# Greketrotny/RayZath

Hardware: AMD Instinct MI355X
Metric: Mrays/s (path segments, primary+secondary) at 1920x1080 depth 8 (higher is better)
Workload: dtype f32; 1 GPU; Cornell box 1920x1080 depth 8; max_depth=8, triangles=16, instances=8, traversal=workgroup-binned, integrator=CPU kernel (parity-checked), pipeline=resident (one kernel per step)

## Files before the change

### rayzath_amd/csrc/hiprz_device.hpp

```cpp
#pragma once
#include <hip/hip_runtime.h>
#include <stdint.h>

#include "hiprz.h"
#include "hiprz_end.hpp"
#include "hiprz_lds.hpp"
#include "hiprz_shard.hpp"

#define RZ_DEV __device__ __forceinline__
#include "hiprz_flat_pick.hpp"
#include "hiprz_deal_pick.hpp"
#include "hiprz_pair_pick.hpp"
#include "hiprz_u8_div.hpp"

namespace hiprz {

#ifndef RZ_FUSED_SHARED_RCP
#define RZ_FUSED_SHARED_RCP 0
#endif
#ifndef RZ_TRACE_SHARED_RCP
#define RZ_TRACE_SHARED_RCP 1
#endif
#ifndef RZ_BATCH_SHARED_RCP
#define RZ_BATCH_SHARED_RCP 1
// ... 230 lines not shown
    if (t <= r.near_ || t >= r.far_) return false;
    t_out = t, b1_out = b1, b2_out = b2, det_out = det;
    return true;
}

struct Instance {
    v3 position, scale, xa, ya, za, bb_min, bb_max;
    uint32_t blas_root, material_base, material_count;
};
RZ_DEV void load_instance_box(const DScene& s, uint32_t i, float4& b0, float4& b1) {
    b0 = s.instances[7 * i + 5];
    b1 = s.instances[7 * i + 6];
}
struct InstanceXform {
    v3 position, scale, xa, ya, za;
    uint32_t blas_root;
    bool unit_scale;
};
RZ_DEV InstanceXform load_instance_xform(const DScene& s, uint32_t i) {
    const float4 a = s.instances[7 * i + 0], b = s.instances[7 * i + 1], c = s.instances[7 * i + 2],
                 d = s.instances[7 * i + 3], e = s.instances[7 * i + 4];
    InstanceXform x;
    x.position = xyz(a), x.blas_root = __float_as_uint(a.w);
    x.scale = xyz(b);
    x.unit_scale = __float_as_uint(d.w) != 0u;
    x.xa = xyz(c), x.ya = xyz(d), x.za = xyz(e);
    return x;
}
RZ_DEV v3 transform_forward(v3 xa, v3 ya, v3 za, v3 v) { return xa * v.x + ya * v.y + za * v.z; }
RZ_DEV v3 transform_backward(v3 xa, v3 ya, v3 za, v3 v) {
    return v3{xa.x * v.x + xa.y * v.y + xa.z * v.z, ya.x * v.x + ya.y * v.y + ya.z * v.z,
              za.x * v.x + za.y * v.y + za.z * v.z};
}
RZ_DEV float to_local(const InstanceXform& x, const Ray& g, Ray& l) {
    l.o = g.o - x.position;
    l.o = transform_backward(x.xa, x.ya, x.za, l.o);
    l.o = l.o / x.scale;
    l.d = transform_backward(x.xa, x.ya, x.za, g.d);
    l.d = l.d / x.scale;
    const float len = magnitude(l.d);
    l.near_ = g.near_ * len;
    l.far_ = g.far_ * len;
    l.d = normalized(l.d);
    return len;
}

struct Hit {
    int32_t instance;
    uint32_t triangle;
    float bx, by;
    bool external;
};


typedef float f2 __attribute__((ext_vector_type(2)));
RZ_DEV float refined_rcp(float d) {
    const float r = __builtin_amdgcn_rcpf(d);
    const float e = __builtin_fmaf(-d, r, 1.0f);
    return __builtin_fmaf(e, r, r);
}
RZ_DEV float div_shared(float n, float d, float y) {
    float q = n * y;
    float r = __builtin_fmaf(-d, q, n);
    q = __builtin_fmaf(r, y, q);
    r = __builtin_fmaf(-d, q, n);
    return __builtin_fmaf(r, y, q);
}
RZ_DEV f2 div_shared2(f2 n, float d, float y) {
    const f2 nd = {-d, -d}, yy = {y, y};
    f2 q = n * yy;
    f2 r = __builtin_elementwise_fma(nd, q, n);
    q = __builtin_elementwise_fma(r, yy, q);
    r = __builtin_elementwise_fma(nd, q, n);
    return __builtin_elementwise_fma(r, yy, q);
}
RZ_DEV bool exponent_in(float x, int lo, int hi) {
    const uint32_t e = (__float_as_uint(x) >> 23) & 0xFFu;
    return (e - uint32_t(lo + 127)) < uint32_t(hi - lo);
}
RZ_DEV bool zero_or_exponent_in(float x, int lo, int hi) {
    return (__float_as_uint(x) & 0x7FFFFFFFu) == 0u || exponent_in(x, lo, hi);
}
#ifdef RZ_PHASE_STATS
static __device__ unsigned long long rz_phase[32];
#define RZ_PHASE(k)                                                                                        \
    do {                                                                                                   \
        const unsigned long long rz_a = __ballot(1);                                                       \
        if (int(__builtin_amdgcn_mbcnt_hi(~0u, __builtin_amdgcn_mbcnt_lo(~0u, 0u))) == __ffsll((long long)rz_a) - 1) { \
            atomicAdd(&rz_phase[2 * (k)], 1ull);                                                           \
            atomicAdd(&rz_phase[2 * (k) + 1], (unsigned long long)__popcll(rz_a));                         \
        }                                                                                                  \
    } while (0)
#else
#define RZ_PHASE(k)
#endif
struct WalkRay {
    v3 o, d, y;
    float near_, far_;
    bool fast;
};
template <bool SHARED_RCP>
RZ_DEV void prepare(WalkRay& r, bool scene_fast) {
    if constexpr (!SHARED_RCP) {
        r.fast = false;
        return;
    }
    r.fast = scene_fast && exponent_in(r.d.x, -40, 2) && exponent_in(r.d.y, -40, 2) && exponent_in(r.d.z, -40, 2) &&
             zero_or_exponent_in(r.o.x, -60, 40) && zero_or_exponent_in(r.o.y, -60, 40) && zero_or_exponent_in(r.o.z, -60, 40);
    r.y = v3{refined_rcp(r.d.x), refined_rcp(r.d.y), refined_rcp(r.d.z)};
}
RZ_DEV float vmin(float a, float b) {
    float r;
    asm("v_min_f32 %0, %1, %2" : "=v"(r) : "v"(a), "v"(b));
    return r;
}
RZ_DEV float vmax(float a, float b) {
    float r;
    asm("v_max_f32 %0, %1, %2" : "=v"(r) : "v"(a), "v"(b));
    return r;
}
RZ_DEV float vmin3(float a, float b, float c) {
    float r;
    asm("v_min3_f32 %0, %1, %2, %3" : "=v"(r) : "v"(a), "v"(b), "v"(c));
    return r;
}
RZ_DEV float vmax3(float a, float b, float c) {
    float r;
    asm("v_max3_f32 %0, %1, %2, %3" : "=v"(r) : "v"(a), "v"(b), "v"(c));
    return r;
}
template <bool SHARED_RCP>
RZ_DEV void box_range_unpacked(float4 b0, float4 b1, const WalkRay& r, float& tmin, float& tmax) {
    if (SHARED_RCP && __all(r.fast)) {
        const float t1 = div_shared(b0.x - r.o.x, r.d.x, r.y.x), t2 = div_shared(b0.y - r.o.x, r.d.x, r.y.x);
        const float t3 = div_shared(b0.z - r.o.y, r.d.y, r.y.y), t4 = div_shared(b0.w - r.o.y, r.d.y, r.y.y);
        const float t5 = div_shared(b1.x - r.o.z, r.d.z, r.y.z), t6 = div_shared(b1.y - r.o.z, r.d.z, r.y.z);
        tmin = vmax3(vmin(t1, t2), vmin(t3, t4), vmin(t5, t6));
        tmax = vmin3(vmax(t1, t2), vmax(t3, t4), vmax(t5, t6));
        return;
    }
    const float t1 = (b0.x - r.o.x) / r.d.x;
    const float t2 = (b0.y - r.o.x) / r.d.x;
    const float t3 = (b0.z - r.o.y) / r.d.y;
    const float t4 = (b0.w - r.o.y) / r.d.y;
    const float t5 = (b1.x - r.o.z) / r.d.z;
    const float t6 = (b1.y - r.o.z) / r.d.z;
    tmin = max_gt(max_gt(min_lt(t1, t2), min_lt(t3, t4)), min_lt(t5, t6));
    tmax = min_lt(min_lt(max_gt(t1, t2), max_gt(t3, t4)), max_gt(t5, t6));
}
RZ_DEV void box_range_fast(float4 b0, float4 b1, const WalkRay& r, float& tmin, float& tmax) {
    const float t1 = div_shared(b0.x - r.o.x, r.d.x, r.y.x), t2 = div_shared(b0.y - r.o.x, r.d.x, r.y.x);
    const float t3 = div_shared(b0.z - r.o.y, r.d.y, r.y.y), t4 = div_shared(b0.w - r.o.y, r.d.y, r.y.y);
    const float t5 = div_shared(b1.x - r.o.z, r.d.z, r.y.z), t6 = div_shared(b1.y - r.o.z, r.d.z, r.y.z);
    tmin = vmax3(vmin(t1, t2), vmin(t3, t4), vmin(t5, t6));
    tmax = vmin3(vmax(t1, t2), vmax(t3, t4), vmax(t5, t6));
}
template <bool SHARED_RCP>
RZ_DEV bool box_hit_unpacked(float4 b0, float4 b1, const WalkRay& r) {
    float tmin, tmax;
    box_range_unpacked<SHARED_RCP>(b0, b1, r, tmin, tmax);
    return !(tmax < r.near_ || tmin > tmax || tmin > r.far_);
}
#ifndef RZ_FILTERED_BOX_TEST
#define RZ_FILTERED_BOX_TEST 1
#endif
RZ_DEV void box_filter(float4 b0, float4 b1, const WalkRay& r, bool& missed, bool& hit) {
    const float a1 = (b0.x - r.o.x) * r.y.x, a2 = (b0.y - r.o.x) * r.y.x;
// ... 209 lines not shown
    while (n != RZ_END) {
        RZ_GUARD(guard);
        const float4 n0 = s.nodes[2 * n], n1 = s.nodes[2 * n + 1];
        RZ_COUNT(box_tests);
        RZ_COUNT(shadow_box_tests);
        if (box_hit<false>(n0, n1, g)) {
            const uint32_t begin = __float_as_uint(n1.z), meta = __float_as_uint(n1.w);
            if (!(meta & HIPRZ_NODE_LEAF)) {
                n = w.descend(begin);
                continue;
            }
            const uint32_t end = begin + (meta & HIPRZ_NODE_COUNT_MASK);
            for (uint32_t i = begin; i < end; ++i) {
                const uint32_t inst = s.tlas_order[i];
                float4 ib0, ib1;
                load_instance_box(s, inst, ib0, ib1);
                RZ_COUNT(box_tests);
        RZ_COUNT(shadow_box_tests);
                if (!box_hit<false>(ib0, ib1, g)) continue;
                const InstanceXform x = load_instance_xform(s, inst);
                WalkRay lr;
                to_local<false>(x, g, lr, scene_fast);
                const uint32_t base = w.mark();
                uint32_t m = x.blas_root;
                while (m != RZ_END) {
                    RZ_GUARD(guard);
                    const float4 m0 = s.nodes[2 * m], m1 = s.nodes[2 * m + 1];
                    RZ_COUNT(box_tests);
        RZ_COUNT(shadow_box_tests);
                    if (box_hit<false>(m0, m1, lr)) {
                        const uint32_t mbegin = __float_as_uint(m1.z), mmeta = __float_as_uint(m1.w);
                        if (!(mmeta & HIPRZ_NODE_LEAF)) {
                            m = w.descend(mbegin);
                            continue;
                        }
                        const uint32_t mend = mbegin + (mmeta & HIPRZ_NODE_COUNT_MASK);
                        for (uint32_t j = mbegin; j < mend; ++j) {
                            const float4 a = s.tris[3 * j], b = s.tris[3 * j + 1], c = s.tris[3 * j + 2];
                            float t, b1, b2, det;
                            RZ_COUNT(tri_tests);
                            RZ_COUNT(shadow_tri_tests);
                            if (tri_hit(xyz(a), xyz(b), xyz(c), lr, t, b1, b2, det)) return 0.0f;
                        }
                    }
                    m = w.next(base);
                }
            }
        } else if (n == s.tlas_root) {
            return 1.0f;
        }
        n = w.next(0u);
    }
    return 1.0f;
}


#define RZ_BIN_NONE 0xFFFFFFFFu
#define RZ_BIN_WIDE 0x80000000u
RZ_DEV uint32_t octet_min(uint32_t v);
struct BinnedLds {
    float* ray;
    uint32_t* hit;
    uint32_t* items;
    uint32_t* bins;
    uint32_t* stacks;
    static constexpr uint32_t kFixedBytes = kBinnedFixedBytes;
    static __host__ uint32_t bytes_host(uint32_t world_entries, uint32_t mesh_entries) {
        return kFixedBytes + (world_entries + mesh_entries) * kBinnedEntryBytes;
    }
    __device__ __forceinline__ explicit BinnedLds(unsigned char* base) {
        ray = reinterpret_cast<float*>(base);
        hit = reinterpret_cast<uint32_t*>(base + 8u * 1024u);
        items = reinterpret_cast<uint32_t*>(base + 13u * 1024u);
        bins = reinterpret_cast<uint32_t*>(base + 14u * 1024u);
        stacks = reinterpret_cast<uint32_t*>(base + kFixedBytes);
    }
};

struct FlatWorld {
    float4 root0, root1;
    uint32_t ids;
    uint32_t count;
    uint32_t wide;
};
RZ_DEV uint32_t wave_uniform(uint32_t v) { return uint32_t(__builtin_amdgcn_readfirstlane(int(v))); }
RZ_DEV float wave_uniform(float v) { return __uint_as_float(wave_uniform(__float_as_uint(v))); }
RZ_DEV float4 wave_uniform(float4 v) { return make_float4(wave_uniform(v.x), wave_uniform(v.y), wave_uniform(v.z), wave_uniform(v.w)); }
RZ_DEV FlatWorld make_flat_world(const DScene& s) {
    FlatWorld fw;
    fw.root0 = fw.root1 = make_float4(0.0f, 0.0f, 0.0f, 0.0f);
    fw.ids = fw.count = fw.wide = 0u;
    if (s.n_instances == 0) return fw;
    fw.root0 = wave_uniform(s.nodes[2 * s.tlas_root]), fw.root1 = wave_uniform(s.nodes[2 * s.tlas_root + 1]);
    const uint32_t begin = __float_as_uint(fw.root1.z);
    fw.count = __float_as_uint(fw.root1.w) & HIPRZ_NODE_COUNT_MASK;
    if (fw.count > 8u) fw.count = 8u;
#pragma unroll
    for (uint32_t k = 0; k < 8u; ++k)
        if (k < fw.count) fw.ids = flat_pack_id(fw.ids, k, wave_uniform(s.tlas_order[begin + k]));
    const uint32_t i = threadIdx.x & 63u;
    bool wide = false;
    if (i < s.n_instances && i < 8u) {
        const uint32_t root = __float_as_uint(s.instances[7 * i].w);
        const uint32_t meta = __float_as_uint(s.nodes[2 * root + 1].w);
        wide = (meta & HIPRZ_NODE_LEAF) != 0u && (meta & HIPRZ_NODE_COUNT_MASK) > 4u;
    }
    fw.wide = uint32_t(__ballot(wide)) & 0xFFu;
    return fw;
}

template <bool COUNT, bool RCP>
RZ_DEV uint32_t pretest_leaf_instances(const DScene& s, const FlatWorld& fw, const WalkRay& g, float (&tm)[8], bool counting, Counters& cnt) {
    uint32_t mask = 0u;
    if (fw.count == 8u && RCP && __all(g.fast)) {
#pragma unroll
        for (uint32_t k = 0; k < 8u; ++k) {
            float4 ib0, ib1;
            load_instance_box(s, flat_id(fw.ids, k), ib0, ib1);
            float tmin, tmax;
            box_range_fast(ib0, ib1, g, tmin, tmax);
            if (counting) { RZ_PHASE(1); RZ_COUNT(box_tests); }
            mask |= uint32_t(!(tmax < g.near_ || tmin > tmax)) << k;
            tm[k] = tmin;
        }
        return mask;
    }
#pragma unroll
    for (uint32_t k = 0; k < 8u; ++k) {
        tm[k] = 0.0f;
        if (k < fw.count) {
            float4 ib0, ib1;
            load_instance_box(s, flat_id(fw.ids, k), ib0, ib1);
            float tmin, tmax;
            box_range_unpacked<RCP>(ib0, ib1, g, tmin, tmax);
            if (counting) { RZ_PHASE(1); RZ_COUNT(box_tests); }
            mask |= uint32_t(!(tmax < g.near_ || tmin > tmax)) << k;
            tm[k] = tmin;
        }
    }
    return mask;
}

RZ_DEV uint32_t lane_pull(uint32_t from_lane, uint32_t v) { return uint32_t(__builtin_amdgcn_ds_bpermute(int(from_lane << 2), int(v))); }
RZ_DEV float lane_pull(uint32_t from_lane, float v) { return __uint_as_float(lane_pull(from_lane, __float_as_uint(v))); }
template <int N>
RZ_DEV uint32_t row_below(uint32_t v) {
    return uint32_t(__builtin_amdgcn_update_dpp(0, int(v), 0x110 + N, 0xF, 0xF, true));
}
RZ_DEV uint32_t wave_inclusive_sum(uint32_t v, uint32_t lane) {
    v += row_below<1>(v), v += row_below<2>(v), v += row_below<4>(v), v += row_below<8>(v);
    const uint32_t r0 = uint32_t(__builtin_amdgcn_readlane(int(v), 15)), r1 = uint32_t(__builtin_amdgcn_readlane(int(v), 31));
    const uint32_t r2 = uint32_t(__builtin_amdgcn_readlane(int(v), 47));
    return v + (lane >= 16u ? r0 : 0u) + (lane >= 32u ? r1 : 0u) + (lane >= 48u ? r2 : 0u);
}
RZ_DEV void dealt_hit(const BinnedLds& lds, uint32_t item, float near_, float len, const LeafBest& best) {
    const uint32_t inst = item >> 8, src = item & 255u;
    lds.ray[6 * 256 + src] = near_ / len;
    lds.ray[7 * 256 + src] = best.far_ / len;
    lds.hit[0 * 256 + src] = best.triangle;
    lds.hit[1 * 256 + src] = best.external ? 1u : 0u;
    lds.hit[2 * 256 + src] = __float_as_uint(best.b1);
    lds.hit[3 * 256 + src] = __float_as_uint(best.b2);
    lds.hit[4 * 256 + src] = inst;
}
template <bool COUNT, bool RCP>
RZ_DEV bool dealt_visit(const DScene& s, const BinnedLds& lds, bool scene_fast, uint32_t slot, bool has_item, Counters& cnt) {
    const uint32_t lane = threadIdx.x & 63u;
    const unsigned char* section = pair_section(s);
    uint32_t item = 0u, rec_off = 0u, begin = 0u, count = 0u, n_pairs = 0u, p = 0u;
    WalkRay lr;
    lr.o = lr.d = lr.y = V3(0.0f, 0.0f, 0.0f), lr.near_ = lr.far_ = 0.0f, lr.fast = false;
    float len = 1.0f;
    bool inner = false;
    if (has_item) {
        item = lds.items[slot];
        const uint32_t inst = item >> 8, src = item & 255u;
        WalkRay w;
        w.o = V3(lds.ray[0 * 256 + src], lds.ray[1 * 256 + src], lds.ray[2 * 256 + src]);
        w.d = V3(lds.ray[3 * 256 + src], lds.ray[4 * 256 + src], lds.ray[5 * 256 + src]);
        w.near_ = lds.ray[6 * 256 + src], w.far_ = lds.ray[7 * 256 + src];
        const InstanceXform x = load_instance_xform(s, inst);
        const float4 n0 = s.nodes[2 * x.blas_root], n1 = s.nodes[2 * x.blas_root + 1];
        inner = (__float_as_uint(n1.w) & HIPRZ_NODE_LEAF) == 0u;
        if (!inner) {
            RZ_PHASE(2);
            len = to_local<RCP>(x, w, lr, scene_fast);
            RZ_PHASE(3);
            RZ_COUNT(box_tests);
            if (box_hit_unpacked<RCP>(n0, n1, lr)) {
                begin = __float_as_uint(n1.z), count = __float_as_uint(n1.w) & HIPRZ_NODE_COUNT_MASK, n_pairs = (count + 1u) >> 1;
// ... 72 lines not shown
        best.far_ = __uint_as_float(nearest);
        best.triangle = won ? won_triangle & ~kDealExternal : 0xFFFFFFFFu;
        best.external = (won_triangle & kDealExternal) != 0u;
        best.b1 = won_b1, best.b2 = won_b2;
        lr.near_ = own_near;
    }
    if (best.triangle != 0xFFFFFFFFu) dealt_hit(lds, item, lr.near_, len, best);
    return inner;
}
template <bool COUNT, bool RCP>
RZ_DEV void binned_visit(const DScene& s, const BinnedLds& lds, uint32_t* mesh_column, bool scene_fast, uint32_t slot, Counters& cnt) {
    RZ_PHASE(2);
    const uint32_t item = lds.items[slot], inst = (item & 0x7FFFFFFFu) >> 8, src = item & 255u;
    WalkRay w;
    w.o = V3(lds.ray[0 * 256 + src], lds.ray[1 * 256 + src], lds.ray[2 * 256 + src]);
    w.d = V3(lds.ray[3 * 256 + src], lds.ray[4 * 256 + src], lds.ray[5 * 256 + src]);
    w.near_ = lds.ray[6 * 256 + src], w.far_ = lds.ray[7 * 256 + src];
    const InstanceXform x = load_instance_xform(s, inst);
    WalkRay lr;
    const float len = to_local<RCP>(x, w, lr, scene_fast);
    const float4 n0 = s.nodes[2 * x.blas_root], n1 = s.nodes[2 * x.blas_root + 1];
    const bool wide = (item & RZ_BIN_WIDE) != 0u;
    if (wide || (__float_as_uint(n1.w) & HIPRZ_NODE_LEAF) != 0u) {
        const uint32_t j = wide ? slot & 7u : 0u;
        RZ_PHASE(3);
        if (j == 0u) { RZ_COUNT(box_tests); }
        LeafBest best;
        best.far_ = lr.far_, best.triangle = 0xFFFFFFFFu, best.b1 = best.b2 = 0.0f, best.external = false;
        if (box_hit_unpacked<RCP>(n0, n1, lr)) {
            const uint32_t begin = __float_as_uint(n1.z), end = begin + (__float_as_uint(n1.w) & HIPRZ_NODE_COUNT_MASK);
            const uint32_t count = end - begin, n_pairs = (count + 1u) >> 1;
            const unsigned char* section = pair_section(s);
            const float2* rec = reinterpret_cast<const float2*>(section + 8u * reinterpret_cast<const uint16_t*>(section)[inst]);
            for (uint32_t p = j; p < n_pairs; p += wide ? 8u : 1u) {
                const float2* q = rec + p * (RZ_PAIR_RECORD_BYTES / 8u);
                const float2 v1x = q[0], v1y = q[1], v1z = q[2], e1x = q[3], e1y = q[4], e1z = q[5], e2x = q[6], e2y = q[7], e2z = q[8];
                const bool has_b = 2u * p + 1u < count;
                const uint32_t i = begin + 2u * p;
                RZ_PHASE(4);
#ifdef RZ_PHASE_STATS
                if (!wide && p >= 1u) { RZ_PHASE(9); }
                if (!wide && p == 1u) {
                    const uint32_t k = uint32_t(__popcll(__ballot(1)));
                    RZ_PHASE(10);
                    if (k <= 12u) { RZ_PHASE(11); } else if (k <= 25u) { RZ_PHASE(12); } else { RZ_PHASE(13); }
                }
#endif
                if constexpr (COUNT) cnt.tri_tests += has_b ? 2u : 1u;
                tri_pair_step(v3p{f2{v1x.x, v1x.y}, f2{v1y.x, v1y.y}, f2{v1z.x, v1z.y}}, v3p{f2{e1x.x, e1x.y}, f2{e1y.x, e1y.y}, f2{e1z.x, e1z.y}},
                              v3p{f2{e2x.x, e2x.y}, f2{e2y.x, e2y.y}, f2{e2z.x, e2z.y}}, i, has_b, lr, best);
            }
        }
        bool mine = best.triangle != 0xFFFFFFFFu;
        if (wide) {
            const uint32_t wide_t = mine ? __float_as_uint(best.far_) : 0xFFFFFFFFu;
            const uint32_t t_min = octet_min(wide_t);
            const bool nearest = wide_t != 0xFFFFFFFFu && wide_t == t_min;
            const uint32_t first = octet_min(nearest ? best.triangle : 0xFFFFFFFFu);
            mine = nearest && best.triangle == first;
        }
        if (mine) {
            lds.ray[6 * 256 + src] = lr.near_ / len;
            lds.ray[7 * 256 + src] = best.far_ / len;
            lds.hit[0 * 256 + src] = best.triangle;
            lds.hit[1 * 256 + src] = best.external ? 1u : 0u;
            lds.hit[2 * 256 + src] = __float_as_uint(best.b1);
            lds.hit[3 * 256 + src] = __float_as_uint(best.b2);
            lds.hit[4 * 256 + src] = inst;
        }
        return;
    }
    LdsStack mesh(mesh_column);
    Hit h;
    if (closest_in_mesh_stack<COUNT, RCP, false>(s, mesh, x.blas_root, lr, h, cnt)) {
        lds.ray[6 * 256 + src] = lr.near_ / len;
        lds.ray[7 * 256 + src] = lr.far_ / len;
        lds.hit[0 * 256 + src] = h.triangle;
        lds.hit[1 * 256 + src] = h.external ? 1u : 0u;
        lds.hit[2 * 256 + src] = __float_as_uint(h.bx);
        lds.hit[3 * 256 + src] = __float_as_uint(h.by);
        lds.hit[4 * 256 + src] = inst;
    }
}

template <bool COUNT, bool RCP>
__device__ __forceinline__ int closest_hit_binned(const DScene& s, unsigned char* workspace, bool active, Ray& ray, Hit& hit,
                                                  Counters& cnt) {
    const uint32_t tid = threadIdx.x;
    BinnedLds lds(workspace);
    hit.instance = -1, hit.triangle = 0, hit.bx = hit.by = 0.0f, hit.external = true;
    if (s.n_instances == 0) return 0;

    lds.ray[0 * 256 + tid] = ray.o.x, lds.ray[1 * 256 + tid] = ray.o.y, lds.ray[2 * 256 + tid] = ray.o.z;
    lds.ray[3 * 256 + tid] = ray.d.x, lds.ray[4 * 256 + tid] = ray.d.y, lds.ray[5 * 256 + tid] = ray.d.z;
    lds.ray[6 * 256 + tid] = ray.near_, lds.ray[7 * 256 + tid] = ray.far_;
    lds.hit[4 * 256 + tid] = 0xFFFFFFFFu;

    LdsStack world(lds.stacks + tid);
    uint32_t* mesh_column = lds.stacks + s.world_stack_entries * 256u + tid;
    const bool sorted = s.n_instances <= 64u;
    WalkRay g;
    g.o = ray.o, g.d = ray.d, g.near_ = ray.near_, g.far_ = ray.far_;
    const bool scene_fast = s.fast_div != 0u;
    prepare<RCP>(g, scene_fast);
    uint32_t n = active ? s.tlas_root : RZ_END;
    uint32_t leaf_i = 0, leaf_end = 0;
    bool root_missed = false;
    uint32_t round = 0u;
    if (tid < 128u) lds.bins[tid] = 0u;
    unsigned long long wide_mask = 0ull;
    if (sorted) {
        const uint32_t k = tid & 63u;
        bool wide = false;
        if (k < s.n_instances) {
            const uint32_t root = __float_as_uint(s.instances[7 * k].w);
            const uint32_t meta = __float_as_uint(s.nodes[2 * root + 1].w);
            wide = (meta & HIPRZ_NODE_LEAF) != 0u && (meta & HIPRZ_NODE_COUNT_MASK) > 4u;
        }
        wide_mask = __ballot(wide);
    }
    __syncthreads();

    uint32_t guard = 0u;
    while (round < (1u << 20)) {
        RZ_PHASE(5);
        uint32_t cand = RZ_BIN_NONE;
        while (true) {
            RZ_GUARD(guard);
            if (leaf_i < leaf_end) {
                const uint32_t inst = s.tlas_order[leaf_i++];
                float4 ib0, ib1;
                load_instance_box(s, inst, ib0, ib1);
                RZ_PHASE(1);
                RZ_COUNT(box_tests);
                if (box_hit_unpacked<RCP>(ib0, ib1, g)) {
                    cand = inst;
                    break;
                }
                continue;
            }
            if (n == RZ_END) break;
            const float4 n0 = s.nodes[2 * n], n1 = s.nodes[2 * n + 1];
            RZ_PHASE(0);
            RZ_COUNT(box_tests);
            if (box_hit_unpacked<RCP>(n0, n1, g)) {
                const uint32_t begin = __float_as_uint(n1.z), meta = __float_as_uint(n1.w);
                if (!(meta & HIPRZ_NODE_LEAF)) {
                    n = world.descend(begin);
                    continue;
                }
                leaf_i = begin, leaf_end = begin + (meta & HIPRZ_NODE_COUNT_MASK);
            } else if (n == s.tlas_root) {
                root_missed = true;
            }
            n = world.next(0u);
        }

        uint32_t* bins = lds.bins + (round & 1u) * 64u;
        uint32_t rank = 0u;
        const uint32_t bin = sorted ? cand : 0u;
        const bool wide_item = cand != RZ_BIN_NONE && cand < 64u && ((wide_mask >> cand) & 1ull) != 0ull;
        if (cand != RZ_BIN_NONE) rank = atomicAdd(&bins[bin], wide_item ? 8u : 1u);
        __syncthreads();
        const uint32_t lane = tid & 63u;
        const uint32_t c = bins[lane];
        const bool wide_bin = ((wide_mask >> lane) & 1ull) != 0ull;
// ... 63 lines not shown
                const uint32_t first = octet_min(nearest ? wide_tri : 0xFFFFFFFFu);
                if (nearest && wide_tri == first) {
                    lds.ray[6 * 256 + src] = visit_near / len;
                    lds.ray[7 * 256 + src] = __uint_as_float(wide_t) / len;
                    lds.hit[0 * 256 + src] = wide_tri;
                    lds.hit[1 * 256 + src] = wide_external ? 1u : 0u;
                    lds.hit[2 * 256 + src] = __float_as_uint(wide_b1);
                    lds.hit[3 * 256 + src] = __float_as_uint(wide_b2);
                    lds.hit[4 * 256 + src] = inst;
                }
            } else {
                LdsStack mesh(mesh_column);
                Hit h;
                if (closest_in_mesh_stack<COUNT, RCP, false>(s, mesh, x.blas_root, lr, h, cnt)) {
                    lds.ray[6 * 256 + src] = lr.near_ / len;
                    lds.ray[7 * 256 + src] = lr.far_ / len;
                    lds.hit[0 * 256 + src] = h.triangle;
                    lds.hit[1 * 256 + src] = h.external ? 1u : 0u;
                    lds.hit[2 * 256 + src] = __float_as_uint(h.bx);
                    lds.hit[3 * 256 + src] = __float_as_uint(h.by);
                    lds.hit[4 * 256 + src] = inst;
                }
            }
        }
        __syncthreads();
        round += 1u;
        g.near_ = lds.ray[6 * 256 + tid];
        g.far_ = lds.ray[7 * 256 + tid];
    }
    ray.o = V3(lds.ray[0 * 256 + tid], lds.ray[1 * 256 + tid], lds.ray[2 * 256 + tid]);
    ray.d = V3(lds.ray[3 * 256 + tid], lds.ray[4 * 256 + tid], lds.ray[5 * 256 + tid]);
    ray.near_ = g.near_, ray.far_ = g.far_;
    const uint32_t inst = lds.hit[4 * 256 + tid];
    if (inst != 0xFFFFFFFFu) {
        hit.instance = int32_t(inst);
        hit.triangle = lds.hit[0 * 256 + tid];
        hit.external = lds.hit[1 * 256 + tid] != 0u;
        hit.bx = __uint_as_float(lds.hit[2 * 256 + tid]);
        hit.by = __uint_as_float(lds.hit[3 * 256 + tid]);
    }
    if (root_missed) return 0;
    return hit.instance >= 0 ? 2 : 1;
}


struct DppShr {
    template <int N>
    __device__ __forceinline__ uint32_t operator()(uint32_t v, FlatShift<N>) const {
        return uint32_t(__builtin_amdgcn_update_dpp(0, int(v), 0x110 + N, 0xF, 0xF, true));
    }
};
template <bool COUNT, bool RCP>
__device__ __forceinline__ int closest_hit_flat(const DScene& s, const FlatWorld& fw, unsigned char* workspace, bool active, Ray& ray, Hit& hit,
                                                Counters& cnt) {
    const uint32_t tid = threadIdx.x;
    BinnedLds lds(workspace);
    hit.instance = -1, hit.triangle = 0, hit.bx = hit.by = 0.0f, hit.external = true;
    if (s.n_instances == 0) return 0;

    lds.ray[0 * 256 + tid] = ray.o.x, lds.ray[1 * 256 + tid] = ray.o.y, lds.ray[2 * 256 + tid] = ray.o.z;
    lds.ray[3 * 256 + tid] = ray.d.x, lds.ray[4 * 256 + tid] = ray.d.y, lds.ray[5 * 256 + tid] = ray.d.z;
    lds.ray[6 * 256 + tid] = ray.near_, lds.ray[7 * 256 + tid] = ray.far_;
    lds.hit[4 * 256 + tid] = 0xFFFFFFFFu;

    uint32_t* mesh_column = lds.stacks + s.world_stack_entries * 256u + tid;
    WalkRay g;
    g.o = ray.o, g.d = ray.d, g.near_ = ray.near_, g.far_ = ray.far_;
    const bool scene_fast = s.fast_div != 0u;
    prepare<RCP>(g, scene_fast);
    bool root_missed = false;
    uint32_t round = 0u;
    float tm[8] = {0.0f, 0.0f, 0.0f, 0.0f, 0.0f, 0.0f, 0.0f, 0.0f};
    uint32_t flat_mask = 0u, flat_next = 0u;
    float flat_near = g.near_;
    if (active) {
        RZ_PHASE(0);
        RZ_COUNT(box_tests);
        if (box_hit_unpacked<RCP>(fw.root0, fw.root1, g)) flat_mask = pretest_leaf_instances<COUNT, RCP>(s, fw, g, tm, true, cnt);
        else root_missed = true;
    }
    if (tid < 128u) lds.bins[tid] = 0u;
    __syncthreads();

    const uint32_t lane = tid & 63u;
    const bool wide_bin = ((fw.wide >> (lane & 7u)) & 1u) != 0u;
    while (round < (1u << 20)) {
        RZ_PHASE(5);
        if (__any(flat_mask != 0u && __float_as_uint(g.near_) != __float_as_uint(flat_near))) {
            if (flat_mask != 0u && __float_as_uint(g.near_) != __float_as_uint(flat_near)) {
                WalkRay t;
                t.o = V3(lds.ray[0 * 256 + tid], lds.ray[1 * 256 + tid], lds.ray[2 * 256 + tid]);
                t.d = V3(lds.ray[3 * 256 + tid], lds.ray[4 * 256 + tid], lds.ray[5 * 256 + tid]);
                t.near_ = g.near_, t.far_ = g.far_;
                prepare<RCP>(t, scene_fast);
                flat_mask = pretest_leaf_instances<COUNT, RCP>(s, fw, t, tm, false, cnt) & flat_from(flat_next);
                flat_near = g.near_;
            }
        }
        const uint32_t cand = flat_pick(fw.ids, tm, g.far_, flat_mask, flat_next);

        uint32_t* bins = lds.bins + (round & 1u) * 64u;
        uint32_t rank = 0u;
        const bool wide_item = cand != kFlatNone && ((fw.wide >> cand) & 1u) != 0u;
        if (cand != kFlatNone) rank = atomicAdd(&bins[cand], wide_item ? 8u : 1u);
        __syncthreads();
        const uint32_t c = bins[lane];
        if (!__any(c != 0u)) break;
        const uint32_t own = flat_pack_bin(c, wide_bin);
        const uint32_t incl = flat_prefix8(own, DppShr{});
        const FlatRound r = flat_round(uint32_t(__builtin_amdgcn_readlane(int(incl), 7)));
#ifdef RZ_PHASE_STATS
        if (!r.split) { RZ_PHASE(6); }
#endif
        const uint32_t before = __shfl(incl - own, int(cand & 7u));
        if (cand != kFlatNone) {
            const uint32_t at = flat_item_slot(r, before, rank, wide_item);
            if (r.split && wide_item) {
#pragma unroll
                for (uint32_t j = 0; j < 8u; ++j) lds.items[at + j] = RZ_BIN_WIDE | (cand << 8) | tid;
            } else {
                lds.items[at] = (cand << 8) | tid;
            }
        }
        if (tid < 64u) lds.bins[((round + 1u) & 1u) * 64u + tid] = 0u;
        __syncthreads();

        const uint32_t slot = (tid - ((blockIdx.x + round) & 3u) * 64u) & 255u;
        const bool has_item = slot < r.n_items;
        bool deal_wave = false;
        if (!r.split && wave_uniform(slot & ~63u) < r.n_items) {
            const bool long_leaf = has_item && ((fw.wide >> (lds.items[has_item ? slot : 0u] >> 8)) & 1u) != 0u;
            const uint32_t owners = uint32_t(__popcll(__ballot(long_leaf)));
            deal_wave = owners != 0u && owners <= kDealMaxOwners;
        }
        bool todo = has_item;
        if (deal_wave) todo = dealt_visit<COUNT, RCP>(s, lds, scene_fast, slot, has_item, cnt);
        if (todo) {
            binned_visit<COUNT, RCP>(s, lds, mesh_column, scene_fast, slot, cnt);
        }
        __syncthreads();
        round += 1u;
        g.near_ = lds.ray[6 * 256 + tid];
        g.far_ = lds.ray[7 * 256 + tid];
    }
    ray.o = V3(lds.ray[0 * 256 + tid], lds.ray[1 * 256 + tid], lds.ray[2 * 256 + tid]);
    ray.d = V3(lds.ray[3 * 256 + tid], lds.ray[4 * 256 + tid], lds.ray[5 * 256 + tid]);
    ray.near_ = g.near_, ray.far_ = g.far_;
    const uint32_t inst = lds.hit[4 * 256 + tid];
    if (inst != 0xFFFFFFFFu) {
        hit.instance = int32_t(inst);
        hit.triangle = lds.hit[0 * 256 + tid];
        hit.external = lds.hit[1 * 256 + tid] != 0u;
        hit.bx = __uint_as_float(lds.hit[2 * 256 + tid]);
        hit.by = __uint_as_float(lds.hit[3 * 256 + tid]);
    }
    if (root_missed) return 0;
    return hit.instance >= 0 ? 2 : 1;
}


struct TopCache {
    const float4* nodes;
    const uint32_t* skip;
    uint32_t count;
    static __host__ uint32_t bytes_host(uint32_t top_count) { return top_count * kTopNodeBytes; }
};
RZ_DEV uint32_t octant_of(v3 d) { return uint32_t(d.z < 0.0f) | (uint32_t(d.y < 0.0f) << 1) | (uint32_t(d.x < 0.0f) << 2); }
RZ_DEV void fetch_node_ordered(const DScene& s, uint32_t n, uint32_t oct, float4& n0, float4& n1, uint32_t& link) {
    const float4* rec = s.nodes64 + 4 * size_t(n);
    n0 = rec[0], n1 = rec[1];
    link = reinterpret_cast<const uint32_t*>(rec + 2)[oct];
}
RZ_DEV bool tri_hit_ordered(v3 v1, v3 edge1, v3 edge2, const WalkRay& r, bool tie_ok, float& t_out, float& b1_out, float& b2_out, float& det_out) {
    const v3 pvec = cross(r.d, edge2);
    float det = dot(edge1, pvec);
    det += float(uint32_t(det > -1.0e-7f) & uint32_t(det < 1.0e-7f)) * 1.0e-7f;
    const float inv_det = 1.0f / det;
    const v3 tvec = r.o - v1;
    const float b1 = dot(tvec, pvec) * inv_det;
    if (b1 < 0.0f || b1 > 1.0f) return false;
    const v3 qvec = cross(tvec, edge1);
    const float b2 = dot(r.d, qvec) * inv_det;
    if (b2 < 0.0f || b1 + b2 > 1.0f) return false;
    const float t = dot(edge2, qvec) * inv_det;
    if (t <= r.near_ || t > r.far_ || (t == r.far_ && !tie_ok)) return false;
    t_out = t, b1_out = b1, b2_out = b2, det_out = det;
    return true;
}
RZ_DEV void fetch_node(const DScene& s, const TopCache& top, uint32_t n, float4& n0, float4& n1, uint32_t& link) {
    if (n < top.count) {
        n0 = top.nodes[2 * n], n1 = top.nodes[2 * n + 1], link = top.skip[n];
    } else {
        n0 = s.nodes[2 * n], n1 = s.nodes[2 * n + 1], link = s.node_skip[n];
    }
}
// ... 1318 lines not shown
```

### rayzath_amd/csrc/hiprz_flat_pick.hpp

```cpp
#pragma once
#include <stdint.h>

#ifndef RZ_DEV
#define RZ_DEV inline
#endif

namespace hiprz {

constexpr uint32_t kFlatNone = 0xFFFFFFFFu;

RZ_DEV uint32_t flat_ctz(uint32_t v) { return uint32_t(__builtin_ctz(v)); }
RZ_DEV uint32_t flat_top_bit(uint32_t v) { return 31u - uint32_t(__builtin_clz(v)); }

RZ_DEV uint32_t flat_pack_id(uint32_t packed, uint32_t k, uint32_t id) { return packed | ((id & 15u) << (4u * k)); }
RZ_DEV uint32_t flat_id(uint32_t packed, uint32_t k) { return (packed >> (4u * k)) & 15u; }
RZ_DEV uint32_t flat_slots(uint32_t count) { return (1u << count) - 1u; }
RZ_DEV uint32_t flat_from(uint32_t next) { return ~((1u << next) - 1u); }

RZ_DEV uint32_t flat_le_mask(const float (&tm)[8], float far_) {
    uint32_t m = 0u;
#pragma unroll
    for (uint32_t k = 0; k < 8u; ++k) m |= uint32_t(!(tm[k] > far_)) << k;
    return m;
}

RZ_DEV uint32_t flat_pick(uint32_t ids, const float (&tm)[8], float far_, uint32_t& mask, uint32_t& next) {
    const uint32_t rest = mask & flat_from(next);
    const uint32_t alive = rest & flat_le_mask(tm, far_);
    if (alive != 0u) {
        const uint32_t k = flat_ctz(alive);
        next = k + 1u;
        return flat_id(ids, k);
    }
    if (rest != 0u) next = flat_top_bit(rest) + 1u;
    mask = 0u;
    return kFlatNone;
}

RZ_DEV uint32_t flat_pack_bin(uint32_t c, bool wide) { return wide ? (c | ((c >> 3) << 21)) : ((c << 12) | (c << 21)); }

template <int N>
struct FlatShift {};
template <class V, class Shr>
RZ_DEV V flat_prefix8(V incl, const Shr& shr) {
    incl += shr(incl, FlatShift<1>{});
    incl += shr(incl, FlatShift<2>{});
    incl += shr(incl, FlatShift<4>{});
    return incl;
}

struct FlatRound {
    uint32_t n_visits, wide_lanes, narrow_lanes, n_items;
    bool split;
};
RZ_DEV FlatRound flat_round(uint32_t totals) {
    FlatRound r;
    r.n_visits = totals >> 21;
    r.wide_lanes = totals & 0xFFFu, r.narrow_lanes = (totals >> 12) & 0x1FFu;
    r.split = r.wide_lanes != 0u && r.wide_lanes + r.narrow_lanes <= 256u;
    r.n_items = r.split ? r.wide_lanes + r.narrow_lanes : r.n_visits;
    return r;
}
RZ_DEV uint32_t flat_item_slot(const FlatRound& r, uint32_t before, uint32_t rank, bool wide_item) {
    if (r.split && wide_item) return (before & 0xFFFu) + rank;
    if (r.split) return r.wide_lanes + ((before >> 12) & 0x1FFu) + rank;
    return (before >> 21) + (wide_item ? rank >> 3 : rank);
}

}
```

### rayzath_amd/csrc/hiprz_launch_shade.hip

```cpp
#include "hiprz_ctx.hpp"
#include "hiprz_kernels.hpp"

#ifndef RZ_PACKET_MINW
#define RZ_PACKET_MINW 4
#endif

namespace hiprz {
namespace {

void sort_after_shading(hiprz_ctx* c, const DFrame& f) {
    launch_sort(c, f.shadow_key != nullptr);
    if (f.shadow_key) launch_shadow_sort(c);
}

template <bool FIRST, bool COUNT>
void launch_shade_t(hiprz_ctx* c, const DFrame& f) {
    const ShadeVariant& v = c->plan.shade;
    const DConfig cfg = make_config(c);
    const dim3 grid(v.grid), block(v.block);
#define RZ_SHADE(L, S) RZ_LAUNCH((rz_shade_kernel<FIRST, COUNT, L, S>), grid, block, v.lds, c->stream, c->dscene, c->dcamera, cfg, f, v.top_n)
    switch (v.shadow) {
        case RZ_SHADOW_COMPAT_DEFER: RZ_SHADE(false, RZ_SHADOW_COMPAT_DEFER); break;
        case RZ_SHADOW_COMPAT: RZ_SHADE(false, RZ_SHADOW_COMPAT); break;
        case RZ_SHADOW_PLAIN:
            if (v.lds_scene) RZ_SHADE(true, RZ_SHADOW_PLAIN);
            else RZ_SHADE(false, RZ_SHADOW_PLAIN);
            break;
        case RZ_SHADOW_NONE:
            if (v.lds_scene) RZ_SHADE(true, RZ_SHADOW_NONE);
            else RZ_SHADE(false, RZ_SHADOW_NONE);
            break;
        case RZ_SHADOW_DEFER: RZ_SHADE(false, RZ_SHADOW_DEFER); break;
        case 1: RZ_SHADE(true, 1); break;
        default: RZ_SHADE(false, 3); break;
    }
#undef RZ_SHADE
    if (v.follow == SHADOWS_NONE) return;
    sort_after_shading(c, f);
    const dim3 sgrid(v.follow_grid), sblock(v.follow_block);
    switch (v.follow) {
        case SHADOWS_PACKET: RZ_LAUNCH((rz_shadow_packet_kernel<FIRST, COUNT, RZ_PACKET_MINW>), sgrid, sblock, v.follow_lds, c->stream, c->dscene, c->dcamera, cfg, f); break;
        case SHADOWS_PACKET_COLOUR: RZ_LAUNCH((rz_shadow_packet_kernel<FIRST, COUNT, RZ_PACKET_MINW, true>), sgrid, sblock, v.follow_lds, c->stream, c->dscene, c->dcamera, cfg, f); break;
        case SHADOWS_COOP3_COLOUR: RZ_LAUNCH((rz_shadow_coop_kernel<FIRST, COUNT, 3, true>), sgrid, sblock, v.follow_lds, c->stream, c->dscene, c->dcamera, cfg, f); break;
        case SHADOWS_COOP4: RZ_LAUNCH((rz_shadow_coop_kernel<FIRST, COUNT, 4>), sgrid, sblock, v.follow_lds, c->stream, c->dscene, c->dcamera, cfg, f); break;
        case SHADOWS_SKIP6: RZ_LAUNCH((rz_shadow_kernel<FIRST, COUNT, 6>), sgrid, sblock, v.follow_lds, c->stream, c->dscene, c->dcamera, cfg, f, v.follow_top_n); break;
        default: RZ_LAUNCH((rz_shadow_kernel<FIRST, COUNT, 4>), sgrid, sblock, v.follow_lds, c->stream, c->dscene, c->dcamera, cfg, f, v.follow_top_n); break;
    }
    join_sort(c);
}

}

void launch_shade(hiprz_ctx* c, const DFrame& f, bool first, bool counted) {
    if (first) counted ? launch_shade_t<true, true>(c, f) : launch_shade_t<true, false>(c, f);
    else counted ? launch_shade_t<false, true>(c, f) : launch_shade_t<false, false>(c, f);
}

}

#ifdef RZ_PHASE_STATS
extern "C" int hiprz_read_shadow_phase_stats(unsigned long long out[32]) {
    (void)hipMemcpyFromSymbol(out, HIP_SYMBOL(hiprz::rz_phase), 256);
    unsigned long long zero[32] = {0};
    (void)hipMemcpyToSymbol(HIP_SYMBOL(hiprz::rz_phase), zero, 256);
    return 0;
}
#endif
```

### rayzath_amd/csrc/hiprz_launch_trace.hip

```cpp
#include "hiprz_ctx.hpp"
#include "hiprz_kernels.hpp"

namespace hiprz {
namespace {

template <bool FIRST, bool COUNT>
void launch_trace_t(hiprz_ctx* c, const DFrame& f) {
    const TraceVariant& t = c->plan.trace;
    const dim3 grid(t.grid), block(t.block);
    if (t.family == TRACE_COMPAT) {
        RZ_LAUNCH((rz_trace_coop_compat_kernel<FIRST, COUNT>), grid, block, t.lds, c->stream, c->dscene, c->dcamera, make_config(c), f);
    } else if (t.family == TRACE_COOP) {
        if (t.waves == 5u && t.one_leaf) RZ_LAUNCH((rz_trace_coop_kernel<FIRST, COUNT, 5, true>), grid, block, t.lds, c->stream, c->dscene, c->dcamera, f);
        else if (t.waves == 5u) RZ_LAUNCH((rz_trace_coop_kernel<FIRST, COUNT, 5>), grid, block, t.lds, c->stream, c->dscene, c->dcamera, f);
        else if (t.waves == 6u) RZ_LAUNCH((rz_trace_coop_kernel<FIRST, COUNT, 6>), grid, block, t.lds, c->stream, c->dscene, c->dcamera, f);
        else if (t.one_leaf) RZ_LAUNCH((rz_trace_coop_kernel<FIRST, COUNT, 4, true>), grid, block, t.lds, c->stream, c->dscene, c->dcamera, f);
        else RZ_LAUNCH((rz_trace_coop_kernel<FIRST, COUNT, 4>), grid, block, t.lds, c->stream, c->dscene, c->dcamera, f);
    } else if (t.family == TRACE_SKIP) {
        if (t.waves == 6u) RZ_LAUNCH((rz_trace_skip_kernel<FIRST, COUNT, 6>), grid, block, t.lds, c->stream, c->dscene, c->dcamera, f, t.top_n);
        else RZ_LAUNCH((rz_trace_skip_kernel<FIRST, COUNT, 4>), grid, block, t.lds, c->stream, c->dscene, c->dcamera, f, t.top_n);
    } else if (t.mode == 4u) {
        RZ_LAUNCH((rz_trace_kernel<FIRST, COUNT, 4, true>), grid, block, t.lds, c->stream, c->dscene, c->dcamera, f);
    } else if (t.mode == 2u) {
        if (t.lds_scene) RZ_LAUNCH((rz_trace_kernel<FIRST, COUNT, 2, true>), grid, block, t.lds, c->stream, c->dscene, c->dcamera, f);
        else RZ_LAUNCH((rz_trace_kernel<FIRST, COUNT, 2, false>), grid, block, t.lds, c->stream, c->dscene, c->dcamera, f);
    } else {
        if (t.lds_scene) RZ_LAUNCH((rz_trace_kernel<FIRST, COUNT, 1, true>), grid, block, t.lds, c->stream, c->dscene, c->dcamera, f);
        else RZ_LAUNCH((rz_trace_kernel<FIRST, COUNT, 1, false>), grid, block, t.lds, c->stream, c->dscene, c->dcamera, f);
    }
}

}

void launch_trace(hiprz_ctx* c, const DFrame& f, bool first, bool counted) {
    if (first) counted ? launch_trace_t<true, true>(c, f) : launch_trace_t<true, false>(c, f);
    else counted ? launch_trace_t<false, true>(c, f) : launch_trace_t<false, false>(c, f);
}

}

#ifdef RZ_PHASE_STATS
extern "C" int hiprz_read_phase_stats(unsigned long long out[32]) {
    (void)hipMemcpyFromSymbol(out, HIP_SYMBOL(hiprz::rz_phase), 256);
    unsigned long long zero[32] = {0};
    (void)hipMemcpyToSymbol(HIP_SYMBOL(hiprz::rz_phase), zero, 256);
    return 0;
}
#endif
```

Measured before the change: 13770 Mrays/s.

## Visit nearest small-leaf instance per-thread before binned traversal

```diff
diff --git a/rayzath_amd/csrc/hiprz_device.hpp b/rayzath_amd/csrc/hiprz_device.hpp
--- a/rayzath_amd/csrc/hiprz_device.hpp
+++ b/rayzath_amd/csrc/hiprz_device.hpp
@@ -336,7 +336,7 @@
     return (__float_as_uint(x) & 0x7FFFFFFFu) == 0u || exponent_in(x, lo, hi);
 }
 #ifdef RZ_PHASE_STATS
-static __device__ unsigned long long rz_phase[32];
+static __device__ unsigned long long rz_phase[40];
 #define RZ_PHASE(k)                                                                                        \
     do {                                                                                                   \
         const unsigned long long rz_a = __ballot(1);                                                       \
@@ -712,6 +712,7 @@
     uint32_t ids;
     uint32_t count;
     uint32_t wide;
+    uint32_t small;
 };
 RZ_DEV uint32_t wave_uniform(uint32_t v) { return uint32_t(__builtin_amdgcn_readfirstlane(int(v))); }
 RZ_DEV float wave_uniform(float v) { return __uint_as_float(wave_uniform(__float_as_uint(v))); }
@@ -719,7 +720,7 @@
 RZ_DEV FlatWorld make_flat_world(const DScene& s) {
     FlatWorld fw;
     fw.root0 = fw.root1 = make_float4(0.0f, 0.0f, 0.0f, 0.0f);
-    fw.ids = fw.count = fw.wide = 0u;
+    fw.ids = fw.count = fw.wide = fw.small = 0u;
     if (s.n_instances == 0) return fw;
     fw.root0 = wave_uniform(s.nodes[2 * s.tlas_root]), fw.root1 = wave_uniform(s.nodes[2 * s.tlas_root + 1]);
     const uint32_t begin = __float_as_uint(fw.root1.z);
@@ -729,13 +730,15 @@
     for (uint32_t k = 0; k < 8u; ++k)
         if (k < fw.count) fw.ids = flat_pack_id(fw.ids, k, wave_uniform(s.tlas_order[begin + k]));
     const uint32_t i = threadIdx.x & 63u;
-    bool wide = false;
+    bool wide = false, small = false;
     if (i < s.n_instances && i < 8u) {
         const uint32_t root = __float_as_uint(s.instances[7 * i].w);
         const uint32_t meta = __float_as_uint(s.nodes[2 * root + 1].w);
         wide = (meta & HIPRZ_NODE_LEAF) != 0u && (meta & HIPRZ_NODE_COUNT_MASK) > 4u;
+        small = (meta & HIPRZ_NODE_LEAF) != 0u && (meta & HIPRZ_NODE_COUNT_MASK) <= 4u;
     }
     fw.wide = uint32_t(__ballot(wide)) & 0xFFu;
+    fw.small = uint32_t(__ballot(small)) & 0xFFu;
     return fw;
 }
 
@@ -974,6 +977,52 @@
         lds.hit[4 * 256 + src] = inst;
     }
 }
+template <bool COUNT, bool RCP>
+RZ_DEV void first_visit(const DScene& s, const BinnedLds& lds, bool scene_fast, uint32_t inst, WalkRay& g, Counters& cnt) {
+    RZ_PHASE(2);
+    const uint32_t src = threadIdx.x;
+    const InstanceXform x = load_instance_xform(s, inst);
+    WalkRay lr;
+    const float len = to_local<RCP>(x, g, lr, scene_fast);
+    const float4 n0 = s.nodes[2 * x.blas_root], n1 = s.nodes[2 * x.blas_root + 1];
+    RZ_PHASE(3);
+    RZ_COUNT(box_tests);
+    LeafBest best;
+    best.far_ = lr.far_, best.triangle = 0xFFFFFFFFu, best.b1 = best.b2 = 0.0f, best.external = false;
+    if (box_hit_unpacked<RCP>(n0, n1, lr)) {
+        const uint32_t begin = __float_as_uint(n1.z), count = __float_as_uint(n1.w) & HIPRZ_NODE_COUNT_MASK, n_pairs = (count + 1u) >> 1;
+        const unsigned char* section = pair_section(s);
+        const float2* rec = reinterpret_cast<const float2*>(section + 8u * reinterpret_cast<const uint16_t*>(section)[inst]);
+        for (uint32_t p = 0u; p < n_pairs; ++p) {
+            const float2* q = rec + p * (RZ_PAIR_RECORD_BYTES / 8u);
+            const float2 v1x = q[0], v1y = q[1], v1z = q[2], e1x = q[3], e1y = q[4], e1z = q[5], e2x = q[6], e2y = q[7], e2z = q[8];
+            const bool has_b = 2u * p + 1u < count;
+            const uint32_t i = begin + 2u * p;
+            RZ_PHASE(4);
+#ifdef RZ_PHASE_STATS
+            if (p >= 1u) {
+                const uint32_t k = uint32_t(__popcll(__ballot(1)));
+                RZ_PHASE(9);
+                RZ_PHASE(10);
+                if (k <= 12u) { RZ_PHASE(11); } else if (k <= 25u) { RZ_PHASE(12); } else { RZ_PHASE(13); }
+            }
+#endif
+            if constexpr (COUNT) cnt.tri_tests += has_b ? 2u : 1u;
+            tri_pair_step(v3p{f2{v1x.x, v1x.y}, f2{v1y.x, v1y.y}, f2{v1z.x, v1z.y}}, v3p{f2{e1x.x, e1x.y}, f2{e1y.x, e1y.y}, f2{e1z.x, e1z.y}},
+                          v3p{f2{e2x.x, e2x.y}, f2{e2y.x, e2y.y}, f2{e2z.x, e2z.y}}, i, has_b, lr, best);
+        }
+    }
+    if (best.triangle != 0xFFFFFFFFu) {
+        g.near_ = lr.near_ / len, g.far_ = best.far_ / len;
+        lds.ray[6 * 256 + src] = g.near_;
+        lds.ray[7 * 256 + src] = g.far_;
+        lds.hit[0 * 256 + src] = best.triangle;
+        lds.hit[1 * 256 + src] = best.external ? 1u : 0u;
+        lds.hit[2 * 256 + src] = __float_as_uint(best.b1);
+        lds.hit[3 * 256 + src] = __float_as_uint(best.b2);
+        lds.hit[4 * 256 + src] = inst;
+    }
+}
 
 template <bool COUNT, bool RCP>
 __device__ __forceinline__ int closest_hit_binned(const DScene& s, unsigned char* workspace, bool active, Ray& ray, Hit& hit,
@@ -1203,6 +1252,21 @@
     if (tid < 128u) lds.bins[tid] = 0u;
     __syncthreads();
 
+#ifdef RZ_PHASE_STATS
+    {
+        uint32_t peek_mask = flat_mask, peek_next = flat_next;
+        const uint32_t peek = flat_pick(fw.ids, tm, g.far_, peek_mask, peek_next);
+        if (peek != kFlatNone) {
+            if (((fw.small >> peek) & 1u) != 0u) { RZ_PHASE(15); } else { RZ_PHASE(16); }
+        }
+    }
+#endif
+    {
+        const uint32_t first = flat_pick_first(fw.ids, tm, g.far_, flat_mask, flat_next, fw.small);
+        if (__any(first != kFlatNone)) {
+            if (first != kFlatNone) first_visit<COUNT, RCP>(s, lds, scene_fast, first, g, cnt);
+        }
+    }
     const uint32_t lane = tid & 63u;
     const bool wide_bin = ((fw.wide >> (lane & 7u)) & 1u) != 0u;
     while (round < (1u << 20)) {
@@ -1232,6 +1296,10 @@
         const FlatRound r = flat_round(uint32_t(__builtin_amdgcn_readlane(int(incl), 7)));
 #ifdef RZ_PHASE_STATS
         if (!r.split) { RZ_PHASE(6); }
+        if (round == 0u) {
+            RZ_PHASE(17);
+            if (!r.split) { RZ_PHASE(18); }
+        }
 #endif
         const uint32_t before = __shfl(incl - own, int(cand & 7u));
         if (cand != kFlatNone) {
diff --git a/rayzath_amd/csrc/hiprz_flat_pick.hpp b/rayzath_amd/csrc/hiprz_flat_pick.hpp
--- a/rayzath_amd/csrc/hiprz_flat_pick.hpp
+++ b/rayzath_amd/csrc/hiprz_flat_pick.hpp
@@ -37,6 +37,20 @@
     return kFlatNone;
 }
 
+RZ_DEV uint32_t flat_pick_first(uint32_t ids, const float (&tm)[8], float far_, uint32_t& mask, uint32_t& next, uint32_t small) {
+    const uint32_t rest = mask & flat_from(next);
+    const uint32_t alive = rest & flat_le_mask(tm, far_);
+    if (alive != 0u) {
+        const uint32_t k = flat_ctz(alive), id = flat_id(ids, k);
+        if (((small >> id) & 1u) == 0u) return kFlatNone;
+        next = k + 1u;
+        return id;
+    }
+    if (rest != 0u) next = flat_top_bit(rest) + 1u;
+    mask = 0u;
+    return kFlatNone;
+}
+
 RZ_DEV uint32_t flat_pack_bin(uint32_t c, bool wide) { return wide ? (c | ((c >> 3) << 21)) : ((c << 12) | (c << 21)); }
 
 template <int N>
diff --git a/rayzath_amd/csrc/hiprz_launch_shade.hip b/rayzath_amd/csrc/hiprz_launch_shade.hip
--- a/rayzath_amd/csrc/hiprz_launch_shade.hip
+++ b/rayzath_amd/csrc/hiprz_launch_shade.hip
@@ -59,10 +59,10 @@
 }
 
 #ifdef RZ_PHASE_STATS
-extern "C" int hiprz_read_shadow_phase_stats(unsigned long long out[32]) {
-    (void)hipMemcpyFromSymbol(out, HIP_SYMBOL(hiprz::rz_phase), 256);
-    unsigned long long zero[32] = {0};
-    (void)hipMemcpyToSymbol(HIP_SYMBOL(hiprz::rz_phase), zero, 256);
+extern "C" int hiprz_read_shadow_phase_stats(unsigned long long out[40]) {
+    (void)hipMemcpyFromSymbol(out, HIP_SYMBOL(hiprz::rz_phase), sizeof(hiprz::rz_phase));
+    unsigned long long zero[40] = {0};
+    (void)hipMemcpyToSymbol(HIP_SYMBOL(hiprz::rz_phase), zero, sizeof(hiprz::rz_phase));
     return 0;
 }
 #endif
diff --git a/rayzath_amd/csrc/hiprz_launch_trace.hip b/rayzath_amd/csrc/hiprz_launch_trace.hip
--- a/rayzath_amd/csrc/hiprz_launch_trace.hip
+++ b/rayzath_amd/csrc/hiprz_launch_trace.hip
@@ -40,10 +40,10 @@
 }
 
 #ifdef RZ_PHASE_STATS
-extern "C" int hiprz_read_phase_stats(unsigned long long out[32]) {
-    (void)hipMemcpyFromSymbol(out, HIP_SYMBOL(hiprz::rz_phase), 256);
-    unsigned long long zero[32] = {0};
-    (void)hipMemcpyToSymbol(HIP_SYMBOL(hiprz::rz_phase), zero, 256);
+extern "C" int hiprz_read_phase_stats(unsigned long long out[40]) {
+    (void)hipMemcpyFromSymbol(out, HIP_SYMBOL(hiprz::rz_phase), sizeof(hiprz::rz_phase));
+    unsigned long long zero[40] = {0};
+    (void)hipMemcpyToSymbol(HIP_SYMBOL(hiprz::rz_phase), zero, sizeof(hiprz::rz_phase));
     return 0;
 }
 #endif
```

Result: faster. 14640 Mrays/s, median of 6 (+6.3%).
